# AHupuJR/REFID

Measured on AMD Instinct MI355X. Metric: interpolated frames/sec (train step) GoPro 256x256 11+1, higher is better.
Workload: dtype f32

## Files before the change

### refid_amd/csrc/wgrad_wino24.hip

```cpp
#include "common.h"
#include "wgrad_args.h"
#include <cstdlib>
#include <cstring>
#include <type_traits>
#include <vector>

#ifndef REFID_W24_ABLATE
#define REFID_W24_ABLATE 0
#endif
#define W24_NO_DMA (REFID_W24_ABLATE == 1 || REFID_W24_ABLATE == 5 || REFID_W24_ABLATE == 6)
#define W24_NO_MFMA (REFID_W24_ABLATE == 2)
#define W24_NO_LDS (REFID_W24_ABLATE == 3 || REFID_W24_ABLATE == 6)
#define W24_NO_BAR (REFID_W24_ABLATE == 4 || REFID_W24_ABLATE == 5 || REFID_W24_ABLATE == 6)

namespace {

__device__ __forceinline__ float w24_fake(float seed) { asm volatile("" : "+v"(seed)); return seed; }

constexpr int IT = 32;
constexpr int TC = 4;
constexpr int GH = 4, GW = 4 * TC;
constexpr int XH = GH + 2, XW = GW + 2;
constexpr int X_BYTES = XH * XW * IT * 4;
constexpr int GS_BYTES = GH * GW * 32 * 4;
// ... 288 lines not shown
        }
    };
    switch (wave) {
        case 0: kloop(std::integral_constant<int, 0>{}); break;
        case 1: kloop(std::integral_constant<int, 1>{}); break;
        case 2: kloop(std::integral_constant<int, 2>{}); break;
        default: kloop(std::integral_constant<int, 3>{}); break;
    }

#pragma unroll
    for (int j = 0; j < 6; ++j) {
        float* sl = a.slabs + ((long long)((split * (DOWN ? 4 : 1) + phase) * NXI + wave * 6 + j) * a.CoP) * a.CiP;
#pragma unroll
        for (int sm = 0; sm < NS; ++sm) {
            const int co = co0 + sm * 32 + li;
#pragma unroll
            for (int qd = 0; qd < 4; ++qd) {
                const int ci = ci0 + 8 * qd + 4 * kh;
                f32x4 vv;
#pragma unroll
                for (int k = 0; k < 4; ++k) vv[k] = acc[j][sm][4 * qd + k];
                f32x4* dst = reinterpret_cast<f32x4*>(sl + (long long)co * a.CiP + ci);
                if (a.accum) vv += *dst;
                *dst = vv;
            }
        }
    }
    if (a.bslabs != nullptr && blockIdx.y == 0 && phase == 0 && wave == 1) {
#pragma unroll
        for (int sm = 0; sm < NS; ++sm) {
            const float tot = bs[sm] + __shfl_xor(bs[sm], 32, 64);
            if (kh == 0) {
                float* dst = a.bslabs + (long long)split * a.CoP + co0 + sm * 32 + li;
                *dst = a.accum ? *dst + tot : tot;
            }
        }
    }
}

constexpr int PAIR_STAGES = 3;
constexpr int PAIR_G0 = 2 * PAIR_STAGES * X_BYTES;
constexpr int PAIR_LDS_BYTES = PAIR_G0 + PAIR_STAGES * 2 * GS_BYTES;

__device__ __forceinline__ int w24_lane_again() {
    int l = __builtin_amdgcn_mbcnt_hi(~0u, __builtin_amdgcn_mbcnt_lo(~0u, 0u));
    asm volatile("" : "+v"(l));
    return l;
}

template <bool DOWN>
__global__ __launch_bounds__(512, 1) void wgrad_wino24_pair_kernel(const W24Args a) {
    constexpr int NS = 2, OT = 32 * NS, XPS = DOWN ? 2 : 1;
    extern __shared__ __attribute__((aligned(16))) char smem[];
    const int tid = threadIdx.x, lane = tid & 63;
    const int wave = __builtin_amdgcn_readfirstlane(tid >> 6);
    const int row = wave & 3, hf = wave >> 2;
    const int li = lane & 31, kh = lane >> 5;
    const int phase = DOWN ? blockIdx.z / a.ncoT : 0, php = phase >> 1, phq = phase & 1;
    const int co0 = (DOWN ? blockIdx.z % a.ncoT : blockIdx.z) * OT, ci0 = (2 * blockIdx.y + hf) * IT;
    const int split = blockIdx.x;
    const int Hin = DOWN ? a.Hin : a.H, Win = DOWN ? a.Win : a.W;

    const bool xFromA = ci0 < a.Ca || ci0 >= a.Ctot;
    const int xld = xFromA ? a.ldA : a.ldB;
    const long long gpixAll = (long long)a.N * a.Ho * a.Wo, xpixAll = (long long)a.N * Hin * Win;
    const int limG = (int)min(gpixAll * a.ldG * 4, 0x7fffffffLL), limX = (int)min(xpixAll * xld * 4, 0x7fffffffLL);
    const int ntAll = a.ntiles * a.groups;
    const int chunk = (ntAll + a.nsplit - 1) / a.nsplit;
    const int p0 = min(split * chunk, ntAll), p1 = min(p0 + chunk, ntAll);

    int qg, qn, qy, qx;
    {
        int t = p0 < ntAll ? p0 : 0;
        qg = t / a.ntiles; t -= qg * a.ntiles;
        qx = t % a.tilesX; t /= a.tilesX;
        qy = t % a.tilesY; qn = t / a.tilesY;
    }
    const int xq = ci0 + (lane & 7) * 4, xt = ci0 + (lane & 31), gq = co0 + (lane & 7) * 4;
    const int xlc = ((lane >> 3) * XPS * xld + (xFromA ? xq : xq - a.Ca)) * 4;
    const int xlt = ((lane >> 5) * XPS * xld + (xFromA ? xt : xt - a.Ca)) * 4;
    const int glc = ((lane >> 3) * a.ldG + gq) * 4;
    const bool fullch = ci0 + IT <= a.Ctot && co0 + OT <= a.Co;
    constexpr int OOB = 0x7ff00000;
    const int xRowB = XPS * Win * xld * 4, gRowB = a.Wo * a.ldG * 4;
    auto x_origin = [&](int n, int ty, int tx) {
        return ((n * Hin + XPS * (ty * GH - a.pad) + php) * Win + XPS * (tx * GW - a.pad) + phq) * xld * 4;
    };
    const float* gPtr = a.g[qg];
    const float* xPtr = xFromA ? a.inA[qg] : a.inB[qg];
    int xTile = x_origin(qn, qy, qx);
    int gTile = ((qn * a.Ho + qy * GH) * a.Wo + qx * GW) * a.ldG * 4;
    const int xr0 = row < 2 ? 2 * row : row + 2, nxr = row < 2 ? 2 : 1;
    const int gr0 = 2 * (row - 2);
    auto request = [&](int st) {
        const int oy0 = qy * GH, ox0 = qx * GW;
        const int iy0 = oy0 - a.pad, ix0 = ox0 - a.pad;
        const __amdgpu_buffer_rsrc_t rsG = __builtin_amdgcn_make_buffer_rsrc(const_cast<float*>(gPtr), 0, limG, 0x00020000);
        const __amdgpu_buffer_rsrc_t rsX = __builtin_amdgcn_make_buffer_rsrc(const_cast<float*>(xPtr), 0, limX, 0x00020000);
        char* xdst = smem + (hf * PAIR_STAGES + st) * X_BYTES;
        char* gdst = smem + PAIR_G0 + st * (2 * GS_BYTES) + hf * GS_BYTES;
        const bool fast = fullch && ix0 >= 0 && ix0 + XW <= a.W && ox0 + GW <= a.Wo && xld * 8 * XPS * 4 < 0x100000 && a.ldG * 8 * 4 < 0x100000;
        if (fast) {
#pragma unroll
            for (int k = 0; k < 2; ++k) {
                if (k < nxr && !W24_NO_DMA) {
                    const int r = xr0 + k;
                    const int base = (unsigned)(iy0 + r) < (unsigned)a.H ? xTile + r * xRowB : OOB;
                    char* dst = xdst + r * (XW * IT * 4);
                    __builtin_amdgcn_raw_ptr_buffer_load_lds(rsX, (lds_ptr24)dst, 16, base + xlc, 0, 0, 0);
                    __builtin_amdgcn_raw_ptr_buffer_load_lds(rsX, (lds_ptr24)(dst + 1024), 16, base + 8 * XPS * xld * 4 + xlc, 0, 0, 0);
                    __builtin_amdgcn_raw_ptr_buffer_load_lds(rsX, (lds_ptr24)(dst + 2048), 4, base + 16 * XPS * xld * 4 + xlt, 0, 0, 0);
                }
            }
#pragma unroll
            for (int k = 0; k < 2; ++k) {
                if (row >= 2 && !W24_NO_DMA) {
                    const int r = gr0 + k;
                    const int base = oy0 + r < a.Ho ? gTile + r * gRowB + hf * 128 : OOB;
                    char* dst = gdst + r * (GW * 32 * 4);
                    __builtin_amdgcn_raw_ptr_buffer_load_lds(rsG, (lds_ptr24)dst, 16, base + glc, 0, 0, 0);
                    __builtin_amdgcn_raw_ptr_buffer_load_lds(rsG, (lds_ptr24)(dst + 1024), 16, base + 8 * a.ldG * 4 + glc, 0, 0, 0);
                }
            }
        } else {
            const int l8 = lane >> 3, l32 = lane >> 5;
            const int xbadq = xq < a.Ctot ? 0 : -1, xbadt = xt < a.Ctot ? 0 : -1;
            const int gbad = gq + hf * 32 < a.Co ? 0 : -1;
            const int cx0 = (unsigned)(ix0 + l8) < (unsigned)a.W ? 0 : -1;
            const int cx1 = (unsigned)(ix0 + 8 + l8) < (unsigned)a.W ? 0 : -1;
            const int cxt = (unsigned)(ix0 + 16 + l32) < (unsigned)a.W ? 0 : -1;
            const int cg0 = ox0 + l8 < a.Wo ? 0 : -1, cg1 = ox0 + 8 + l8 < a.Wo ? 0 : -1;
#pragma unroll
            for (int k = 0; k < 2; ++k) {
                if (k < nxr && !W24_NO_DMA) {
                    const int r = xr0 + k;
                    const int rbad = (unsigned)(iy0 + r) < (unsigned)a.H ? 0 : -1;
                    const int base = xTile + r * xRowB;
                    char* dst = xdst + r * (XW * IT * 4);
                    __builtin_amdgcn_raw_ptr_buffer_load_lds(rsX, (lds_ptr24)dst, 16, (base + xlc) | xbadq | rbad | cx0, 0, 0, 0);
                    __builtin_amdgcn_raw_ptr_buffer_load_lds(rsX, (lds_ptr24)(dst + 1024), 16,
                                                             (base + 8 * XPS * xld * 4 + xlc) | xbadq | rbad | cx1, 0, 0, 0);
                    __builtin_amdgcn_raw_ptr_buffer_load_lds(rsX, (lds_ptr24)(dst + 2048), 4,
                                                             (base + 16 * XPS * xld * 4 + xlt) | xbadt | rbad | cxt, 0, 0, 0);
                }
            }
#pragma unroll
            for (int k = 0; k < 2; ++k) {
                if (row >= 2 && !W24_NO_DMA) {
                    const int r = gr0 + k;
                    const int rbad = oy0 + r < a.Ho ? 0 : -1;
                    const int base = gTile + r * gRowB + hf * 128;
                    char* dst = gdst + r * (GW * 32 * 4);
                    __builtin_amdgcn_raw_ptr_buffer_load_lds(rsG, (lds_ptr24)dst, 16, (base + glc) | gbad | rbad | cg0, 0, 0, 0);
                    __builtin_amdgcn_raw_ptr_buffer_load_lds(rsG, (lds_ptr24)(dst + 1024), 16,
                                                             (base + 8 * a.ldG * 4 + glc) | gbad | rbad | cg1, 0, 0, 0);
                }
            }
        }
        if (REFID_W24_ABLATE == 7) return;
        qx += 1;
        if (qx != a.tilesX) {
            xTile += GW * XPS * xld * 4;
            gTile += GW * a.ldG * 4;
        } else {
            qx = 0;
            qy += 1;
            if (qy == a.tilesY) {
                qy = 0;
                qn += 1;
                if (qn == a.N) {
                    qn = 0;
                    qg = min(qg + 1, a.groups - 1);
                    gPtr = a.g[qg];
                    xPtr = xFromA ? a.inA[qg] : a.inB[qg];
                }
            }
            xTile = x_origin(qn, qy, 0);
            gTile = (qn * a.Ho + qy * GH) * a.Wo * a.ldG * 4;
        }
    };

    f32x16 acc[6][NS];
#pragma unroll
    for (int j = 0; j < 6; ++j)
#pragma unroll
        for (int sm = 0; sm < NS; ++sm)
#pragma unroll
            for (int r = 0; r < 16; ++r) acc[j][sm][r] = 0.f;

    static_assert(X_BYTES % 256 == 0 && (PAIR_STAGES * X_BYTES) / 256 < 256 && (PAIR_STAGES * 2 * GS_BYTES) / 256 < 256,
                  "ds_read2st64 offset range");
    lds_cf24* xe = (lds_cf24*)(smem + hf * PAIR_STAGES * X_BYTES) + (2 * kh) * (XW * IT) + li;
    lds_cf24* ge = (lds_cf24*)(smem + PAIR_G0) + (2 * kh) * (GW * 32) + li;
    lds_cf24* xb[4] = {xe, xe + IT, xe + 2 * IT, xe + 3 * IT};
    lds_cf24* gb[4] = {ge, ge + 32, ge + 2 * 32, ge + 3 * 32};
    asm volatile("" : "+v"(xb[0]), "+v"(xb[1]), "+v"(xb[2]), "+v"(xb[3]), "+v"(xe));
    asm volatile("" : "+v"(gb[0]), "+v"(gb[1]), "+v"(gb[2]), "+v"(gb[3]));

    auto kloop = [&](auto TI) {
        constexpr int I = decltype(TI)::value;
        using R = W24Row<I>;
        float bs[NS];
#pragma unroll
        for (int sm = 0; sm < NS; ++sm) bs[sm] = 0.f;
        auto tile = [&](auto ST) {
            constexpr int XO = decltype(ST)::value * (X_BYTES / 4), GO = decltype(ST)::value * (2 * GS_BYTES / 4);
            lds_cf24* xbb[4] = {xb[0] + XO, xb[1] + XO, xb[2] + XO, xb[3] + XO};
            lds_cf24* gbb[4] = {gb[0] + GO, gb[1] + GO, gb[2] + GO, gb[3] + GO};
            f32x2 t[6], p4, p5;
#pragma unroll
            for (int s = 0; s < TC; s += 2) {
                R::x_rows(xbb, s, t);
                if (s == 0) {
                    const f32x2 a01 = R::x_rows01(xe + XO);
                    t[0] = w24_pair<0, 0>(a01, t[4]);
                    t[1] = w24_pair<1, 0>(a01, t[5]);
                } else {
                    t[0] = w24_pair<1, 0>(p4, t[4]);
                    t[1] = w24_pair<1, 0>(p5, t[5]);
                }
                p4 = t[4]; p5 = t[5];
                f32x2 v[6];
                R::v_cols(t, v);
#pragma unroll
                for (int sm = 0; sm < NS; ++sm) {
                    f32x2 x[4], z[6];
                    R::g_rows(gbb, s, sm, x);
                    R::z_cols(x, z);
                    if constexpr (I == 1) bs[sm] += z[1][0] + z[1][1];
#pragma unroll
                    for (int h = 0; h < 2; ++h)
#pragma unroll
                        for (int j = 0; j < 6; ++j) {
                            if (W24_NO_MFMA) { asm volatile("" :: "v"(v[j][h]), "v"(z[j][h])); continue; }
                            acc[j][sm] = __builtin_amdgcn_mfma_f32_32x32x2f32(v[j][h], z[j][h], acc[j][sm], 0, 0, 0);
                        }
                }
            }
        };
        const int n = p1 - p0;
        auto step = [&](auto ST, int j) {
            constexpr int S = decltype(ST)::value;
            if (j + 1 < n) __builtin_amdgcn_s_waitcnt(I < 2 ? 0x0F76 : 0x0F77);
            else __builtin_amdgcn_s_waitcnt(0x0F70);
            if (!W24_NO_BAR) __builtin_amdgcn_s_barrier();
            __builtin_amdgcn_sched_barrier(0);
            if (j + 2 < n) request((S + 2) % PAIR_STAGES);
            tile(ST);
        };
        if (n > 0) request(0);
        if (n > 1) request(1);
        int j = 0;
        for (; j + 3 <= n; j += 3) {
            step(std::integral_constant<int, 0>{}, j);
            step(std::integral_constant<int, 1>{}, j + 1);
            step(std::integral_constant<int, 2>{}, j + 2);
        }
        if (j < n) {
            step(std::integral_constant<int, 0>{}, j);
            if (j + 1 < n) step(std::integral_constant<int, 1>{}, j + 1);
        }
        if constexpr (I == 1) {
            if (a.bslabs != nullptr && blockIdx.y == 0 && hf == 0 && phase == 0) {
                const int le = w24_lane_again();
#pragma unroll
                for (int sm = 0; sm < NS; ++sm) {
                    const float tot = bs[sm] + __shfl_xor(bs[sm], 32, 64);
                    if ((le >> 5) == 0) {
                        float* dst = a.bslabs + (long long)split * a.CoP + co0 + sm * 32 + (le & 31);
                        *dst = a.accum ? *dst + tot : tot;
                    }
                }
            }
        }
    };
    switch (row) {
        case 0: kloop(std::integral_constant<int, 0>{}); break;
        case 1: kloop(std::integral_constant<int, 1>{}); break;
        case 2: kloop(std::integral_constant<int, 2>{}); break;
        default: kloop(std::integral_constant<int, 3>{}); break;
    }

    const int le = w24_lane_again(), lie = le & 31, khe = le >> 5;
#pragma unroll
    for (int j = 0; j < 6; ++j) {
        float* sl = a.slabs + ((long long)((split * (DOWN ? 4 : 1) + phase) * NXI + row * 6 + j) * a.CoP) * a.CiP;
#pragma unroll
        for (int sm = 0; sm < NS; ++sm) {
            const int co = co0 + sm * 32 + lie;
#pragma unroll
            for (int qd = 0; qd < 4; ++qd) {
                const int ci = ci0 + 8 * qd + 4 * khe;
                f32x4 vv;
#pragma unroll
                for (int k = 0; k < 4; ++k) vv[k] = acc[j][sm][4 * qd + k];
                f32x4* dst = reinterpret_cast<f32x4*>(sl + (long long)co * a.CiP + ci);
                if (a.accum) vv += *dst;
                *dst = vv;
            }
        }
    }
}

struct W24rArgs {
    const float* slabs; const float* bslabs; float* dw; float* db;
    int nsplit, Co, Ci, CoP, CiP, iBase, iTotal, perGroup;
    int nsplitW;
    int down;
};

__device__ __forceinline__ void w24_fold_body(const float* __restrict__ slabs, float* __restrict__ part, long long slabFloats,
                                              int nsplit, int S, int piece, int s) {
    const long long off = ((long long)piece * 256 + threadIdx.x) * 4;
    if (off >= slabFloats) return;
    const f32x4* p = reinterpret_cast<const f32x4*>(slabs + off);
    const long long st4 = slabFloats / 4;
    f32x4 a0 = {0.f, 0.f, 0.f, 0.f}, a1 = a0;
    int k = s;
    for (; k + S < nsplit; k += 2 * S) { a0 += p[k * st4]; a1 += p[(k + S) * st4]; }
    if (k < nsplit) a0 += p[k * st4];
    *reinterpret_cast<f32x4*>(part + (long long)s * slabFloats + off) = a0 + a1;
}
__global__ __launch_bounds__(256) void wgrad_wino24_fold_kernel(const float* __restrict__ slabs, float* __restrict__ part,
                                                                long long slabFloats, int nsplit, int S) {
    w24_fold_body(slabs, part, slabFloats, nsplit, S, blockIdx.x, blockIdx.y);
}

constexpr int FOLD_BATCH = 96;
struct FoldJob { const float* slabs; float* part; long long slabFloats; int nsplit, S; };
struct FoldBatch { FoldJob job[FOLD_BATCH]; int blk0[FOLD_BATCH + 1]; int n; };
static_assert(sizeof(FoldBatch) <= 4096, "kernel-argument block");
__global__ __launch_bounds__(256) void wgrad_fold_batch_kernel(const FoldBatch b) {
    int j = 0;
    for (int k = 1; k < b.n; ++k) j = (int)blockIdx.x >= b.blk0[k] ? k : j;
    const FoldJob& f = b.job[j];
    const int blk = (int)blockIdx.x - b.blk0[j];
    const int pieces = (int)((f.slabFloats / 4 + 255) / 256);
    w24_fold_body(f.slabs, f.part, f.slabFloats, f.nsplit, f.S, blk % pieces, blk / pieces);
}
thread_local std::vector<FoldJob> fold_queue;

__device__ __forceinline__ void w24_reduce_body(const W24rArgs& a, const int blk, float* part) {
    const long long plane = (long long)a.CoP * a.CiP;
    const long long slabStride = NXI * plane;
    const int lpe = a.perGroup, eb = 256 / lpe;
    const int el = threadIdx.x % eb, sub = threadIdx.x / eb;
    const long long e = (long long)blk * eb + el;
    const bool live = e < (long long)a.Co * a.Ci;
    const int ci = live ? (int)(e % a.Ci) : 0, co = live ? (int)(e / a.Ci) : 0;
    {
        const float* p = a.slabs + (long long)co * a.CiP + ci;
        float u[NXI];
#pragma unroll
        for (int x = 0; x < NXI; ++x) u[x] = 0.f;
        if (live) {
            for (int k = sub; k < a.nsplitW; k += lpe) {
#pragma unroll
                for (int x = 0; x < NXI; ++x) u[x] += p[k * slabStride + x * plane];
            }
        }
        if (lpe > 1) {
#pragma unroll
            for (int x = 0; x < NXI; ++x) part[threadIdx.x * (NXI + 1) + x] = u[x];
            __syncthreads();
            if (sub == 0) {
                for (int s2 = 1; s2 < lpe; ++s2) {
#pragma unroll
                    for (int x = 0; x < NXI; ++x) u[x] += part[(s2 * eb + el) * (NXI + 1) + x];
                }
            }
        }
        if (live && sub == 0) {
            constexpr float c4 = 0.25f, c6 = 1.f / 6.f, c12 = 1.f / 12.f, c24 = 1.f / 24.f;
            float dg[9];
#pragma unroll
            for (int pp = 0; pp < 3; ++pp) {
                float t[6];
#pragma unroll
                for (int j = 0; j < 6; ++j) {
                    const float m = 0.5f * (u[6 + j] + u[12 + j]), d = 0.5f * (u[6 + j] - u[12 + j]);
                    t[j] = pp == 0 ? u[j] + m : (pp == 1 ? d : m + u[18 + j]);
                }
                const float s12 = t[1] + t[2], d21 = t[2] - t[1], s34 = t[3] + t[4], d34 = t[3] - t[4];
                dg[pp * 3 + 0] = c4 * t[0] - c6 * s12 + c24 * s34;
                dg[pp * 3 + 1] = c6 * d21 + c12 * d34;
                dg[pp * 3 + 2] = c6 * (s34 - s12) + t[5];
            }
            float* dst = a.dw + ((long long)co * a.iTotal + a.iBase + ci) * 9;
#pragma unroll
            for (int k = 0; k < 9; ++k) dst[k] += dg[k];
        }
    }
    if (a.db != nullptr && blk == 0) {
        for (int c2 = threadIdx.x; c2 < a.Co; c2 += 256) {
            float s = 0.f;
            for (int k = 0; k < a.nsplit; ++k) s += a.bslabs[(long long)k * a.CoP + c2];
            a.db[c2] += s;
        }
    }
}

__global__ __launch_bounds__(256) void wgrad_wino24_reduce_kernel(const W24rArgs a) {
    __shared__ float part[256 * (NXI + 1)];
    w24_reduce_body(a, blockIdx.x, part);
}

__device__ __forceinline__ void w24_reduce_down_body(const W24rArgs& a, const int blk) {
    const long long plane = (long long)a.CoP * a.CiP;
    const long long slabStride = 4 * NXI * plane;
    const long long gid = (long long)blk * 256 + threadIdx.x;
    const long long e = gid >> 2;
    const int ph = (int)(gid & 3);
    const bool live = e < (long long)a.Co * a.Ci;
    const int ci = live ? (int)(e % a.Ci) : 0, co = live ? (int)(e / a.Ci) : 0;
    if (live) {
        const float* p = a.slabs + (long long)co * a.CiP + ci + ph * NXI * plane;
        float u[NXI];
#pragma unroll
        for (int x = 0; x < NXI; ++x) u[x] = 0.f;
        for (int k = 0; k < a.nsplitW; ++k) {
#pragma unroll
            for (int x = 0; x < NXI; ++x) u[x] += p[k * slabStride + x * plane];
        }
        constexpr float c4 = 0.25f, c6 = 1.f / 6.f, c12 = 1.f / 12.f, c24 = 1.f / 24.f;
        float* dst = a.dw + ((long long)co * a.iTotal + a.iBase + ci) * 16;
#pragma unroll
        for (int pp = 0; pp < 3; ++pp) {
            const int ky = 2 * pp + (ph >> 1) - 1;
            float t[6];
#pragma unroll
            for (int j = 0; j < 6; ++j) {
                const float m = 0.5f * (u[6 + j] + u[12 + j]), d = 0.5f * (u[6 + j] - u[12 + j]);
                t[j] = pp == 0 ? u[j] + m : (pp == 1 ? d : m + u[18 + j]);
            }
            const float s12 = t[1] + t[2], d21 = t[2] - t[1], s34 = t[3] + t[4], d34 = t[3] - t[4];
            const float r3[3] = {c4 * t[0] - c6 * s12 + c24 * s34, c6 * d21 + c12 * d34, c6 * (s34 - s12) + t[5]};
            if (ky < 0 || ky > 3) continue;
#pragma unroll
            for (int q = 0; q < 3; ++q) {
                const int kx = 2 * q + (ph & 1) - 1;
                if (kx >= 0 && kx <= 3) dst[ky * 4 + kx] += r3[q];
            }
        }
    }
    if (a.db != nullptr && blk == 0) {
        for (int c2 = threadIdx.x; c2 < a.Co; c2 += 256) {
            float sacc = 0.f;
            for (int k = 0; k < a.nsplit; ++k) sacc += a.bslabs[(long long)k * a.CoP + c2];
            a.db[c2] += sacc;
        }
    }
}

__global__ __launch_bounds__(256) void wgrad_wino24_reduce_down_kernel(const W24rArgs a) { w24_reduce_down_body(a, blockIdx.x); }

struct W24rBatch { W24rArgs job[REFID_FINISH_BATCH]; int blk0[REFID_FINISH_BATCH + 1]; int n; };
static_assert(sizeof(W24rBatch) <= 4096, "kernel-argument block");
__global__ __launch_bounds__(256) void wgrad_wino24_reduce_batch_kernel(const W24rBatch b) {
    __shared__ float part[256 * (NXI + 1)];
    int j = 0;
    for (int k = 1; k < b.n; ++k) j = (int)blockIdx.x >= b.blk0[k] ? k : j;
    const int blk = (int)blockIdx.x - b.blk0[j];
    if (b.job[j].down) w24_reduce_down_body(b.job[j], blk);
    else w24_reduce_body(b.job[j], blk, part);
}

struct W24rQueued { W24rArgs r; int nblocks; };
thread_local std::vector<W24rQueued> w24_queue;

struct Geo24 { int ncoT, nciT, tilesX, tilesY, ntiles, nsplit, CoP, CiP; };

int ns_of(const refid_wgrad_desc* d) { return d->c_o <= 32 ? 1 : 2; }
bool is_down(const refid_wgrad_desc* d) { return d->kh == 4; }

Geo24 geo24_of(const refid_wgrad_desc* d) {
    Geo24 g;
    const int OT = 32 * ns_of(d);
    g.ncoT = cdiv(d->c_o, OT);
    const int ci_geo = (d->phase != 0) ? d->i_total - d->i_base : d->c_a + d->c_b;
    g.nciT = cdiv(ci_geo > d->c_a + d->c_b ? ci_geo : d->c_a + d->c_b, IT);
    g.tilesX = cdiv(d->wo, GW);
    g.tilesY = cdiv(d->ho, GH);
    g.ntiles = g.tilesX * g.tilesY * d->n;
    const char* wgsEnv = getenv("REFID_W24_WGS");
    const int wgs = wgsEnv ? atoi(wgsEnv) : 512;
    int want = cdiv(ns_of(d) == 1 ? wgs * 3 / 2 : wgs, g.ncoT * g.nciT * (is_down(d) ? 4 : 1));
    if (want >= 8) want = want / 8 * 8;
    if (want < 1) want = 1;
    if (want > g.ntiles) want = g.ntiles;
    g.nsplit = want;
    g.CoP = g.ncoT * OT;
    g.CiP = g.nciT * IT;
    return g;
}

int pair_mode() { const char* e = getenv("REFID_W24_PAIR"); return e ? atoi(e) : 1; }
bool pair_fits(const refid_wgrad_desc* d, const Geo24& g) { return ns_of(d) == 2 && g.nciT % 2 == 0; }

}

int refid_slab_fold_count(long long slabFloats, int nsplit) {
    if (nsplit < 2) return 0;
    const long long pieces = (slabFloats / 4 + 255) / 256;
    int S = (int)((2048 + pieces - 1) / pieces);
    if (S > 16) S = 16;
    if (S >= nsplit) S = nsplit / 2;
    return S < 1 ? 1 : S;
}
int refid_launch_slab_fold(const float* slabs, float* part, long long slabFloats, int nsplit, int S, hipStream_t st) {
    static const bool batch_folds = !(getenv("REFID_FOLD_BATCH") && getenv("REFID_FOLD_BATCH")[0] == '0');
    if (batch_folds && refid_finish_defer_now()) {
        fold_queue.push_back({slabs, part, slabFloats, nsplit, S});
        return 0;
    }
    hipLaunchKernelGGL(wgrad_wino24_fold_kernel, dim3((unsigned)((slabFloats / 4 + 255) / 256), S), dim3(256), 0, st, slabs, part,
                       slabFloats, nsplit, S);
    REFID_LAUNCH_CHECK("wgrad_slab_fold");
    return 0;
}

int refid_slab_fold_flush(hipStream_t st) {
    size_t at = 0;
    while (at < fold_queue.size()) {
        FoldBatch b;
        memset(&b, 0, sizeof(b));
        int n = 0;
        long long blk = 0;
        for (; n < FOLD_BATCH && at < fold_queue.size(); ++n, ++at) {
            const FoldJob& f = fold_queue[at];
            const long long nb = ((f.slabFloats / 4 + 255) / 256) * f.S;
            if (n > 0 && blk + nb > 0x3fffffffLL) break;
            b.job[n] = f;
            b.blk0[n] = (int)blk;
            blk += nb;
        }
        b.blk0[n] = (int)blk; b.n = n;
        hipLaunchKernelGGL(wgrad_fold_batch_kernel, dim3((unsigned)blk), dim3(256), 0, st, b);
        if (hipGetLastError() != hipSuccess) { fold_queue.clear(); refid_set_error("wgrad_fold_batch: launch failed"); return 1; }
    }
    fold_queue.clear();
    return 0;
}

int refid_wino24_finish_flush(hipStream_t st) {
    size_t at = 0;
    while (at < w24_queue.size()) {
        W24rBatch b;
        memset(&b, 0, sizeof(b));
        int n = 0, blk = 0;
        for (; n < REFID_FINISH_BATCH && at < w24_queue.size(); ++n, ++at) {
            b.job[n] = w24_queue[at].r;
            b.blk0[n] = blk;
            blk += w24_queue[at].nblocks;
        }
        b.blk0[n] = blk; b.n = n;
        hipLaunchKernelGGL(wgrad_wino24_reduce_batch_kernel, dim3(blk), dim3(256), 0, st, b);
        if (hipGetLastError() != hipSuccess) { w24_queue.clear(); refid_set_error("wgrad_wino24_reduce_batch: launch failed"); return 1; }
    }
    w24_queue.clear();
    return 0;
}

namespace {
long long slab_floats(const refid_wgrad_desc* d, const Geo24& g) { return (long long)(is_down(d) ? 4 : 1) * NXI * g.CoP * g.CiP; }
}

size_t refid_wgrad_wino24_workspace_bytes(const refid_wgrad_desc* d) {
    const Geo24 g = geo24_of(d);
    const long long slab = slab_floats(d, g);
    return ((size_t)g.nsplit * slab + (size_t)g.nsplit * g.CoP + (size_t)refid_slab_fold_count(slab, g.nsplit) * slab) * sizeof(float);
}

int refid_wgrad_wino24_launch(const refid_wgrad_desc* d, hipStream_t st) {
    static std::atomic<unsigned long long> attr_done{0}, attr_done1{0}, attr_done2{0}, attr_done3{0};
    if (int rc = refid_lds_attr_once(attr_done, &wgrad_wino24_kernel<2, false>, lds24_bytes(2), "wgrad_wino24")) return rc;
    if (int rc = refid_lds_attr_once(attr_done1, &wgrad_wino24_kernel<1, false>, lds24_bytes(1), "wgrad_wino24<1>")) return rc;
    if (int rc = refid_lds_attr_once(attr_done2, &wgrad_wino24_kernel<2, true>, lds24_bytes(2), "wgrad_wino24<down>")) return rc;
    if (int rc = refid_lds_attr_once(attr_done3, &wgrad_wino24_kernel<1, true>, lds24_bytes(1), "wgrad_wino24<1, down>")) return rc;
    static std::atomic<unsigned long long> attr_done4{0}, attr_done5{0};
    if (int rc = refid_lds_attr_once(attr_done4, &wgrad_wino24_pair_kernel<false>, PAIR_LDS_BYTES, "wgrad_wino24<pair>")) return rc;
    if (int rc = refid_lds_attr_once(attr_done5, &wgrad_wino24_pair_kernel<true>, PAIR_LDS_BYTES, "wgrad_wino24<pair, down>")) return rc;
    const Geo24 g = geo24_of(d);
    const bool down = is_down(d);
    const long long slab = slab_floats(d, g);
    const int pmode = pair_mode();
    const bool pair = pmode != 0 && pair_fits(d, g);
    REFID_CHECK(pair || pmode != 2, "wgrad (Winograd 2x4 tiles): REFID_W24_PAIR=2, but this launch takes the four-wave form "
                                    "(c_o <= 32 or an odd number of input-channel tiles)");
    if (down)
        REFID_CHECK(d->kw == 4 && d->stride == 2 && d->pad == 1 && d->h % 2 == 0 && d->w % 2 == 0 && d->ho == d->h / 2 && d->wo == d->w / 2,
                    "wgrad (algo 7): a 4x4 stride-2 pad-1 conv over an even-sized input");
    REFID_CHECK(d->c_b == 0 || d->c_a % IT == 0, "wgrad (Winograd 2x4 tiles): c_a must be a multiple of %d for two sources", IT);
    REFID_CHECK(d->ld_g % 4 == 0 && d->ld_a % 4 == 0 && (d->c_b == 0 || d->ld_b % 4 == 0) && d->c_o % 4 == 0 &&
                    d->c_a % 4 == 0 && d->c_b % 4 == 0,
                "wgrad (Winograd 2x4 tiles): pitches and channel counts must be multiples of 4 floats (16-byte LDS-DMA pieces)");
    {
        const long long lim = 0x7fffffffLL;
        REFID_CHECK((long long)d->n * d->ho * d->wo * d->ld_g * 4 < lim && (long long)d->n * d->h * d->w * d->ld_a * 4 < lim &&
                        (d->c_b == 0 || (long long)d->n * d->h * d->w * d->ld_b * 4 < lim),
                    "wgrad (Winograd 2x4 tiles): tensor too large for 32-bit buffer offsets (use algo 0)");
    }
    W24Args a;
    const int ngrp = d->groups > 1 ? d->groups : 1;
    REFID_CHECK(ngrp <= REFID_WGRAD_MAX_GROUPS, "wgrad: at most %d grouped time steps", REFID_WGRAD_MAX_GROUPS);
    for (int k = 0; k < REFID_WGRAD_MAX_GROUPS; ++k) {
        const bool on = k > 0 && k < ngrp;
        a.g[k] = k == 0 ? d->g : (on ? d->g_more[k - 1] : d->g);
        a.inA[k] = k == 0 ? d->in_a : (on ? d->in_a_more[k - 1] : d->in_a);
        a.inB[k] = k == 0 ? d->in_b : (on ? d->in_b_more[k - 1] : d->in_b);
        REFID_CHECK(a.g[k] && a.inA[k] && (d->c_b == 0 || a.inB[k]), "wgrad: null tensor pointer in group %d", k);
        REFID_CHECK(((uintptr_t)a.g[k] | (uintptr_t)a.inA[k] | (uintptr_t)(d->c_b ? a.inB[k] : nullptr)) % 16 == 0,
                    "wgrad (Winograd 2x4 tiles): tensors must be 16-byte aligned (group %d)", k);
    }
    a.groups = ngrp;
    a.ldG = d->ld_g; a.Co = d->c_o;
    a.ldA = d->ld_a; a.ldB = d->ld_b;
    a.Ca = d->c_a; a.Ctot = d->c_a + d->c_b;
    a.slabs = d->slabs;
    a.bslabs = d->db ? d->slabs + (size_t)g.nsplit * slab : nullptr;
    a.N = d->n; a.H = d->h; a.W = d->w; a.Ho = d->ho; a.Wo = d->wo; a.pad = d->pad;
    a.Hin = d->h; a.Win = d->w; a.ncoT = g.ncoT;
    if (down) { a.H = d->ho; a.W = d->wo; a.pad = 1; }
    a.tilesX = g.tilesX; a.tilesY = g.tilesY; a.ntiles = g.ntiles; a.nsplit = g.nsplit;
    a.CoP = g.CoP; a.CiP = g.CiP;
    a.accum = (d->phase == 2);
    if (d->phase != 3) {
        if (pair) {
            if (down)
                hipLaunchKernelGGL((wgrad_wino24_pair_kernel<true>), dim3(g.nsplit, g.nciT / 2, 4 * g.ncoT), dim3(512), PAIR_LDS_BYTES, st, a);
            else
                hipLaunchKernelGGL((wgrad_wino24_pair_kernel<false>), dim3(g.nsplit, g.nciT / 2, g.ncoT), dim3(512), PAIR_LDS_BYTES, st, a);
        } else if (down) {
            if (ns_of(d) == 1)
                hipLaunchKernelGGL((wgrad_wino24_kernel<1, true>), dim3(g.nsplit, g.nciT, 4 * g.ncoT), dim3(256), lds24_bytes(1), st, a);
            else
                hipLaunchKernelGGL((wgrad_wino24_kernel<2, true>), dim3(g.nsplit, g.nciT, 4 * g.ncoT), dim3(256), lds24_bytes(2), st, a);
        } else if (ns_of(d) == 1)
            hipLaunchKernelGGL((wgrad_wino24_kernel<1, false>), dim3(g.nsplit, g.nciT, g.ncoT), dim3(256), lds24_bytes(1), st, a);
        else
            hipLaunchKernelGGL((wgrad_wino24_kernel<2, false>), dim3(g.nsplit, g.nciT, g.ncoT), dim3(256), lds24_bytes(2), st, a);
        REFID_LAUNCH_CHECK("wgrad_wino24");
    }
    if (d->phase == 1 || d->phase == 2) return 0;
    W24rArgs r;
    r.slabs = a.slabs; r.bslabs = a.bslabs; r.dw = d->dw; r.db = d->db;
    r.nsplit = g.nsplit; r.Co = d->o_real;
    int nred = g.nsplit;
    if (const int S = refid_slab_fold_count(slab, g.nsplit)) {
        const long long slabFloats = slab;
        float* part = d->slabs + (size_t)g.nsplit * slab + (size_t)g.nsplit * g.CoP;
        if (int rc = refid_launch_slab_fold(a.slabs, part, slabFloats, g.nsplit, S, st)) return rc;
        r.slabs = part;
        nred = S;
    }
    r.Ci = (d->phase == 0 && a.Ctot < d->i_total - d->i_base) ? a.Ctot : d->i_total - d->i_base;
    r.CoP = g.CoP; r.CiP = g.CiP; r.iBase = d->i_base; r.iTotal = d->i_total;
    const long long total = (long long)r.Co * r.Ci;
    int lpe = 1;
    while (lpe < 16 && (long long)lpe * 2 * total <= 65536 && lpe * 2 <= nred) lpe *= 2;
    r.perGroup = lpe;
    r.nsplitW = nred;
    r.down = down ? 1 : 0;
    if (refid_finish_defer_now()) {
        for (const W24rQueued& q : w24_queue)
            if (q.r.dw == r.dw && q.r.iBase == r.iBase) {
                if (int rc = refid_slab_fold_flush(st)) return rc;
                if (int rc = refid_wino24_finish_flush(st)) return rc;
                break;
            }
        w24_queue.push_back({r, down ? (int)((total * 4 + 255) / 256) : (int)((total + 256 / lpe - 1) / (256 / lpe))});
        return 0;
    }
    if (down) {
        hipLaunchKernelGGL(wgrad_wino24_reduce_down_kernel, dim3((int)((total * 4 + 255) / 256)), dim3(256), 0, st, r);
        REFID_LAUNCH_CHECK("wgrad_wino24_reduce_down");
        return 0;
    }
    hipLaunchKernelGGL(wgrad_wino24_reduce_kernel, dim3((int)((total + 256 / lpe - 1) / (256 / lpe))), dim3(256), 0, st, r);
    REFID_LAUNCH_CHECK("wgrad_wino24_reduce");
    return 0;
}
```

Measured before the change: 506.8.

## Add dedicated Winograd kernel and reduce path for stride-2 4x4 down-conv weight grads

Adds a separate weight-gradient kernel for the 4x4 stride-2 downsampling convolution. It uses a different Winograd decomposition with 6-row output tiles, 20 transform points and its own input/gradient transforms, plus a matching reduce body that inverts the transform into the 4x4 kernel taps. It is enabled by default through REFID_W24_DOWN and bypasses the pair kernel for these layers. The aim is fewer MFMA and transform operations per down-conv tile, paid for with a new code path, a different slab layout, a larger workspace and some numerical risk.

```diff
diff --git a/refid_amd/csrc/wgrad_wino24.hip b/refid_amd/csrc/wgrad_wino24.hip
--- a/refid_amd/csrc/wgrad_wino24.hip
+++ b/refid_amd/csrc/wgrad_wino24.hip
@@ -614,6 +614,296 @@
     }
 }
 
+constexpr int DGH = 6, DXH = DGH + 1;
+constexpr int DX_BYTES = DXH * XW * IT * 4;
+constexpr int DGS_BYTES = DGH * GW * 32 * 4;
+constexpr int down_lds_bytes(int ns) { return 2 * (DX_BYTES + ns * DGS_BYTES); }
+constexpr int NXD = 20;
+
+template <int I>
+struct W24DownRow {
+    using B = W24Row<I>;
+    static constexpr int XR = XW * IT, GR = GW * 32, GSUB = DGH * GW * 32;
+    static __device__ __forceinline__ void x_rows(lds_cf24* const (&xb)[4], int s, f32x2 (&t)[5]) {
+#pragma unroll
+        for (int c = 0; c < 4; ++c) {
+            const int col = 4 * s + 1 + c;
+            lds_cf24* p = xb[col & 3] + (col & ~3) * IT;
+            const f32x2 a = f32x2{p[B::XA * XR], p[B::XA * XR + 4 * IT]};
+            const f32x2 b = f32x2{p[B::XB * XR], p[B::XB * XR + 4 * IT]};
+            t[1 + c] = B::x_comb(a, b);
+        }
+    }
+    static __device__ __forceinline__ float x_row0(lds_cf24* xe) { return B::x_comb(xe[B::XA * XR], xe[B::XB * XR]); }
+    static __device__ __forceinline__ void g_rows(lds_cf24* const (&gb)[4], int s, int sub, f32x2 (&x)[4]) {
+#pragma unroll
+        for (int c = 0; c < 4; ++c) {
+            const int col = 4 * s + c;
+            lds_cf24* p = gb[col & 3] + sub * GSUB + (col & ~3) * 32;
+            if constexpr (I == 0) x[c] = f32x2{p[0], p[4 * 32]};
+            else if constexpr (I == 3) x[c] = f32x2{p[2 * GR], p[2 * GR + 4 * 32]};
+            else {
+                const f32x2 g0 = f32x2{p[0], p[4 * 32]}, g1 = f32x2{p[GR], p[GR + 4 * 32]}, g2 = f32x2{p[2 * GR], p[2 * GR + 4 * 32]};
+                x[c] = I == 1 ? (g0 + g2) + g1 : (g0 + g2) - g1;
+            }
+        }
+    }
+    static __device__ __forceinline__ void v_cols(const f32x2 (&t)[5], f32x2 (&v)[5]) {
+        const f32x2 d31 = t[3] - t[1];
+        v[0] = 2.f * (t[0] - t[2]) + d31;
+        v[1] = (t[3] - t[2]) - 2.f * t[1];
+        v[2] = 2.f * t[1] + (-3.f * t[2] + t[3]);
+        v[3] = d31;
+        v[4] = (t[4] - t[2]) - 2.f * d31;
+    }
+    static __device__ __forceinline__ void z_cols(const f32x2 (&x)[4], f32x2 (&z)[5]) {
+        const f32x2 e = x[0] + x[2], o = x[1] + x[3], e4 = 4.f * x[2] + x[0], o4 = 4.f * x[3] + x[1];
+        z[0] = x[0]; z[1] = e + o; z[2] = e - o; z[3] = 2.f * o4 + e4; z[4] = x[3];
+    }
+};
+
+template <int NS>
+__global__ __launch_bounds__(256, 2) void wgrad_wino24_down_kernel(const W24Args a) {
+    constexpr int OT = 32 * NS, XPS = 2;
+    constexpr int G0 = 2 * DX_BYTES, GST_BYTES = NS * DGS_BYTES;
+    extern __shared__ __attribute__((aligned(16))) char smem[];
+    const int tid = threadIdx.x, lane = tid & 63;
+    const int wave = __builtin_amdgcn_readfirstlane(tid >> 6);
+    const int li = lane & 31, kh = lane >> 5;
+    const int phase = blockIdx.z / a.ncoT, php = phase >> 1, phq = phase & 1;
+    const int co0 = (blockIdx.z % a.ncoT) * OT, ci0 = blockIdx.y * IT;
+    const int split = blockIdx.x;
+    const int Hin = a.Hin, Win = a.Win;
+
+    const bool xFromA = ci0 < a.Ca || ci0 >= a.Ctot;
+    const int xld = xFromA ? a.ldA : a.ldB;
+    const long long gpixAll = (long long)a.N * a.Ho * a.Wo, xpixAll = (long long)a.N * Hin * Win;
+    const int limG = (int)min(gpixAll * a.ldG * 4, 0x7fffffffLL), limX = (int)min(xpixAll * xld * 4, 0x7fffffffLL);
+    const int ntAll = a.ntiles * a.groups;
+    const int chunk = (ntAll + a.nsplit - 1) / a.nsplit;
+    const int p0 = min(split * chunk, ntAll), p1 = min(p0 + chunk, ntAll);
+
+    int qg, qn, qy, qx;
+    {
+        int t = p0 < ntAll ? p0 : 0;
+        qg = t / a.ntiles; t -= qg * a.ntiles;
+        qx = t % a.tilesX; t /= a.tilesX;
+        qy = t % a.tilesY; qn = t / a.tilesY;
+    }
+    const int xq = ci0 + (lane & 7) * 4, xt = ci0 + (lane & 31), gq = co0 + (lane & 7) * 4;
+    const int xlc = ((lane >> 3) * XPS * xld + (xFromA ? xq : xq - a.Ca)) * 4;
+    const int xlt = ((lane >> 5) * XPS * xld + (xFromA ? xt : xt - a.Ca)) * 4;
+    const int glc = ((lane >> 3) * a.ldG + gq) * 4;
+    const bool fullch = ci0 + IT <= a.Ctot && co0 + OT <= a.Co;
+    constexpr int OOB = 0x7ff00000;
+    const int xRowB = XPS * Win * xld * 4, gRowB = a.Wo * a.ldG * 4;
+    auto x_origin = [&](int n, int ty, int tx) {
+        return ((n * Hin + XPS * (ty * DGH - php) + php) * Win + XPS * (tx * GW - phq) + phq) * xld * 4;
+    };
+    const float* gPtr = a.g[qg];
+    const float* xPtr = xFromA ? a.inA[qg] : a.inB[qg];
+    int xTile = x_origin(qn, qy, qx);
+    int gTile = ((qn * a.Ho + qy * DGH) * a.Wo + qx * GW) * a.ldG * 4;
+    const int q0 = NS == 2 ? 3 * wave : wave, nq = NS == 2 ? 3 : (wave < 3 ? 1 : 3);
+    auto request = [&](int buf) {
+        const int oy0 = qy * DGH, ox0 = qx * GW;
+        const int iy0 = oy0 - php, ix0 = ox0 - phq;
+        const __amdgpu_buffer_rsrc_t rsG = __builtin_amdgcn_make_buffer_rsrc(const_cast<float*>(gPtr), 0, limG, 0x00020000);
+        const __amdgpu_buffer_rsrc_t rsX = __builtin_amdgcn_make_buffer_rsrc(const_cast<float*>(xPtr), 0, limX, 0x00020000);
+        char* xdst = smem + buf * DX_BYTES;
+        char* gdst = smem + G0 + buf * GST_BYTES;
+        const bool fast = fullch && ix0 >= 0 && ix0 + XW - 1 <= a.W && ox0 + GW <= a.Wo && xld * 8 * XPS * 4 < 0x100000 && a.ldG * 8 * 4 < 0x100000;
+        if (fast) {
+#pragma unroll
+            for (int k = 0; k < 2; ++k) {
+                const int r = wave + 4 * k;
+                if (r < DXH) {
+                    const int base = (unsigned)(iy0 + r) < (unsigned)a.H ? xTile + r * xRowB : OOB;
+                    char* dst = xdst + r * (XW * IT * 4);
+                    __builtin_amdgcn_raw_ptr_buffer_load_lds(rsX, (lds_ptr24)dst, 16, base + xlc, 0, 0, 0);
+                    __builtin_amdgcn_raw_ptr_buffer_load_lds(rsX, (lds_ptr24)(dst + 1024), 16, base + 8 * XPS * xld * 4 + xlc, 0, 0, 0);
+                    __builtin_amdgcn_raw_ptr_buffer_load_lds(rsX, (lds_ptr24)(dst + 2048), 4, base + 16 * XPS * xld * 4 + xlt, 0, 0, 0);
+                }
+            }
+#pragma unroll
+            for (int k = 0; k < 3; ++k) {
+                if (k < nq) {
+                    const int q = q0 + k, r = q % DGH, sub = q / DGH;
+                    const int base = oy0 + r < a.Ho ? gTile + r * gRowB + sub * 128 : OOB;
+                    char* dst = gdst + sub * DGS_BYTES + r * (GW * 32 * 4);
+                    __builtin_amdgcn_raw_ptr_buffer_load_lds(rsG, (lds_ptr24)dst, 16, base + glc, 0, 0, 0);
+                    __builtin_amdgcn_raw_ptr_buffer_load_lds(rsG, (lds_ptr24)(dst + 1024), 16, base + 8 * a.ldG * 4 + glc, 0, 0, 0);
+                }
+            }
+        } else {
+            const int l8 = lane >> 3, l32 = lane >> 5;
+            const int xbadq = xq < a.Ctot ? 0 : -1, xbadt = xt < a.Ctot ? 0 : -1;
+            const int gbad0 = gq < a.Co ? 0 : -1, gbad1 = gq + 32 < a.Co ? 0 : -1;
+            const int cx0 = (unsigned)(ix0 + l8) < (unsigned)a.W ? 0 : -1;
+            const int cx1 = (unsigned)(ix0 + 8 + l8) < (unsigned)a.W ? 0 : -1;
+            const int cxt = (unsigned)(ix0 + 16 + l32) < (unsigned)a.W ? 0 : -1;
+            const int cg0 = ox0 + l8 < a.Wo ? 0 : -1, cg1 = ox0 + 8 + l8 < a.Wo ? 0 : -1;
+#pragma unroll
+            for (int k = 0; k < 2; ++k) {
+                const int r = wave + 4 * k;
+                if (r < DXH) {
+                    const int rbad = (unsigned)(iy0 + r) < (unsigned)a.H ? 0 : -1;
+                    const int base = xTile + r * xRowB;
+                    char* dst = xdst + r * (XW * IT * 4);
+                    __builtin_amdgcn_raw_ptr_buffer_load_lds(rsX, (lds_ptr24)dst, 16, (base + xlc) | xbadq | rbad | cx0, 0, 0, 0);
+                    __builtin_amdgcn_raw_ptr_buffer_load_lds(rsX, (lds_ptr24)(dst + 1024), 16,
+                                                             (base + 8 * XPS * xld * 4 + xlc) | xbadq | rbad | cx1, 0, 0, 0);
+                    __builtin_amdgcn_raw_ptr_buffer_load_lds(rsX, (lds_ptr24)(dst + 2048), 4,
+                                                             (base + 16 * XPS * xld * 4 + xlt) | xbadt | rbad | cxt, 0, 0, 0);
+                }
+            }
+#pragma unroll
+            for (int k = 0; k < 3; ++k) {
+                if (k < nq) {
+                    const int q = q0 + k, r = q % DGH, sub = q / DGH;
+                    const int rbad = oy0 + r < a.Ho ? 0 : -1;
+                    const int base = gTile + r * gRowB + sub * 128;
+                    const int gbad = sub ? gbad1 : gbad0;
+                    char* dst = gdst + sub * DGS_BYTES + r * (GW * 32 * 4);
+                    __builtin_amdgcn_raw_ptr_buffer_load_lds(rsG, (lds_ptr24)dst, 16, (base + glc) | gbad | rbad | cg0, 0, 0, 0);
+                    __builtin_amdgcn_raw_ptr_buffer_load_lds(rsG, (lds_ptr24)(dst + 1024), 16,
+                                                             (base + 8 * a.ldG * 4 + glc) | gbad | rbad | cg1, 0, 0, 0);
+                }
+            }
+        }
+        qx += 1;
+        if (qx != a.tilesX) {
+            xTile += GW * XPS * xld * 4;
+            gTile += GW * a.ldG * 4;
+        } else {
+            qx = 0;
+            qy += 1;
+            if (qy == a.tilesY) {
+                qy = 0;
+                qn += 1;
+                if (qn == a.N) {
+                    qn = 0;
+                    qg = min(qg + 1, a.groups - 1);
+                    gPtr = a.g[qg];
+                    xPtr = xFromA ? a.inA[qg] : a.inB[qg];
+                }
+            }
+            xTile = x_origin(qn, qy, 0);
+            gTile = (qn * a.Ho + qy * DGH) * a.Wo * a.ldG * 4;
+        }
+    };
+
+    f32x16 acc[5][NS];
+#pragma unroll
+    for (int j = 0; j < 5; ++j)
+#pragma unroll
+        for (int sm = 0; sm < NS; ++sm)
+#pragma unroll
+            for (int r = 0; r < 16; ++r) acc[j][sm][r] = 0.f;
+    float bs[NS];
+#pragma unroll
+    for (int sm = 0; sm < NS; ++sm) bs[sm] = 0.f;
+
+    static_assert(DX_BYTES % 256 == 0 && DGS_BYTES % 256 == 0 && (DX_BYTES + 3 * XW * IT * 4 + 16 * IT * 4) / 256 < 256 &&
+                      (GST_BYTES + NS * DGS_BYTES) / 256 < 256, "ds_read2st64 offset range");
+    lds_cf24* xe = (lds_cf24*)smem + (3 * kh) * (XW * IT) + li;
+    lds_cf24* ge = (lds_cf24*)(smem + G0) + (3 * kh) * (GW * 32) + li;
+    lds_cf24* xb[4] = {xe, xe + IT, xe + 2 * IT, xe + 3 * IT};
+    lds_cf24* gb[4] = {ge, ge + 32, ge + 2 * 32, ge + 3 * 32};
+    asm volatile("" : "+v"(xb[0]), "+v"(xb[1]), "+v"(xb[2]), "+v"(xb[3]), "+v"(xe));
+    asm volatile("" : "+v"(gb[0]), "+v"(gb[1]), "+v"(gb[2]), "+v"(gb[3]));
+
+    auto kloop = [&](auto TI) {
+        constexpr int I = decltype(TI)::value;
+        using R = W24DownRow<I>;
+        auto tile = [&](auto BUF) {
+            constexpr int XO = decltype(BUF)::value * (DX_BYTES / 4), GO = decltype(BUF)::value * (GST_BYTES / 4);
+            lds_cf24* xbb[4] = {xb[0] + XO, xb[1] + XO, xb[2] + XO, xb[3] + XO};
+            lds_cf24* gbb[4] = {gb[0] + GO, gb[1] + GO, gb[2] + GO, gb[3] + GO};
+            f32x2 t[5], p4;
+#pragma unroll
+            for (int s = 0; s < TC; s += 2) {
+                R::x_rows(xbb, s, t);
+                if (s == 0) {
+                    const float c0 = R::x_row0(xe + XO);
+                    t[0] = w24_pair<0, 0>(f32x2{c0, c0}, t[4]);
+                } else {
+                    t[0] = w24_pair<1, 0>(p4, t[4]);
+                }
+                p4 = t[4];
+                f32x2 v[5];
+                R::v_cols(t, v);
+#pragma unroll
+                for (int sm = 0; sm < NS; ++sm) {
+                    f32x2 x[4], z[5];
+                    R::g_rows(gbb, s, sm, x);
+                    R::z_cols(x, z);
+                    if constexpr (I == 1) bs[sm] += z[1][0] + z[1][1];
+#pragma unroll
+                    for (int h = 0; h < 2; ++h)
+#pragma unroll
+                        for (int j = 0; j < 5; ++j)
+                            acc[j][sm] = __builtin_amdgcn_mfma_f32_32x32x2f32(v[j][h], z[j][h], acc[j][sm], 0, 0, 0);
+                }
+            }
+        };
+        auto sync = [&] {
+            __builtin_amdgcn_s_waitcnt(0x0F70);
+            __builtin_amdgcn_s_barrier();
+            __builtin_amdgcn_sched_barrier(0);
+        };
+        const int npairs = (p1 - p0) >> 1;
+        if (p0 < p1) request(0);
+        for (int i = 0; i < npairs; ++i) {
+            sync();
+            request(1);
+            tile(std::integral_constant<int, 0>{});
+            sync();
+            if (p0 + 2 * i + 2 < p1) request(0);
+            tile(std::integral_constant<int, 1>{});
+        }
+        if ((p1 - p0) & 1) {
+            sync();
+            tile(std::integral_constant<int, 0>{});
+        }
+    };
+    switch (wave) {
+        case 0: kloop(std::integral_constant<int, 0>{}); break;
+        case 1: kloop(std::integral_constant<int, 1>{}); break;
+        case 2: kloop(std::integral_constant<int, 2>{}); break;
+        default: kloop(std::integral_constant<int, 3>{}); break;
+    }
+
+#pragma unroll
+    for (int j = 0; j < 5; ++j) {
+        float* sl = a.slabs + ((long long)((split * 4 + phase) * NXD + wave * 5 + j) * a.CoP) * a.CiP;
+#pragma unroll
+        for (int sm = 0; sm < NS; ++sm) {
+            const int co = co0 + sm * 32 + li;
+#pragma unroll
+            for (int qd = 0; qd < 4; ++qd) {
+                const int ci = ci0 + 8 * qd + 4 * kh;
+                f32x4 vv;
+#pragma unroll
+                for (int k = 0; k < 4; ++k) vv[k] = acc[j][sm][4 * qd + k];
+                f32x4* dst = reinterpret_cast<f32x4*>(sl + (long long)co * a.CiP + ci);
+                if (a.accum) vv += *dst;
+                *dst = vv;
+            }
+        }
+    }
+    if (a.bslabs != nullptr && blockIdx.y == 0 && phase == 0 && wave == 1) {
+#pragma unroll
+        for (int sm = 0; sm < NS; ++sm) {
+            const float tot = bs[sm] + __shfl_xor(bs[sm], 32, 64);
+            if (kh == 0) {
+                float* dst = a.bslabs + (long long)split * a.CoP + co0 + sm * 32 + li;
+                *dst = a.accum ? *dst + tot : tot;
+            }
+        }
+    }
+}
+
 struct W24rArgs {
     const float* slabs; const float* bslabs; float* dw; float* db;
     int nsplit, Co, Ci, CoP, CiP, iBase, iTotal, perGroup;
@@ -764,7 +1054,53 @@
     }
 }
 
-__global__ __launch_bounds__(256) void wgrad_wino24_reduce_down_kernel(const W24rArgs a) { w24_reduce_down_body(a, blockIdx.x); }
+__device__ __forceinline__ void w24_reduce_down23_body(const W24rArgs& a, const int blk) {
+    const long long plane = (long long)a.CoP * a.CiP;
+    const long long slabStride = 4 * NXD * plane;
+    const long long gid = (long long)blk * 256 + threadIdx.x;
+    const long long e = gid >> 2;
+    const int ph = (int)(gid & 3);
+    const bool live = e < (long long)a.Co * a.Ci;
+    const int ci = live ? (int)(e % a.Ci) : 0, co = live ? (int)(e / a.Ci) : 0;
+    if (live) {
+        const float* p = a.slabs + (long long)co * a.CiP + ci + ph * NXD * plane;
+        float u[NXD];
+#pragma unroll
+        for (int x = 0; x < NXD; ++x) u[x] = 0.f;
+        for (int k = 0; k < a.nsplitW; ++k) {
+#pragma unroll
+            for (int x = 0; x < NXD; ++x) u[x] += p[k * slabStride + x * plane];
+        }
+        constexpr float c6 = 1.f / 6.f;
+        float* dst = a.dw + ((long long)co * a.iTotal + a.iBase + ci) * 16;
+#pragma unroll
+        for (int pp = 0; pp < 2; ++pp) {
+            const int ky = 2 * pp + 1 - (ph >> 1);
+            float t[5];
+#pragma unroll
+            for (int j = 0; j < 5; ++j) {
+                const float m = 0.5f * (u[5 + j] + u[10 + j]), d = 0.5f * (u[5 + j] - u[10 + j]);
+                t[j] = pp == 0 ? u[j] + m : d + u[15 + j];
+            }
+            const float r2[2] = {0.5f * (t[0] - t[1]) + c6 * (t[3] - t[2]), (c6 * t[2] - 0.5f * t[1]) + (2.f * c6 * t[3] + t[4])};
+            const int kx = 1 - (ph & 1);
+            dst[ky * 4 + kx] += r2[0];
+            dst[ky * 4 + kx + 2] += r2[1];
+        }
+    }
+    if (a.db != nullptr && blk == 0) {
+        for (int c2 = threadIdx.x; c2 < a.Co; c2 += 256) {
+            float sacc = 0.f;
+            for (int k = 0; k < a.nsplit; ++k) sacc += a.bslabs[(long long)k * a.CoP + c2];
+            a.db[c2] += sacc;
+        }
+    }
+}
+
+__global__ __launch_bounds__(256) void wgrad_wino24_reduce_down_kernel(const W24rArgs a) {
+    if (a.down == 2) w24_reduce_down23_body(a, blockIdx.x);
+    else w24_reduce_down_body(a, blockIdx.x);
+}
 
 struct W24rBatch { W24rArgs job[REFID_FINISH_BATCH]; int blk0[REFID_FINISH_BATCH + 1]; int n; };
 static_assert(sizeof(W24rBatch) <= 4096, "kernel-argument block");
@@ -773,7 +1109,8 @@
     int j = 0;
     for (int k = 1; k < b.n; ++k) j = (int)blockIdx.x >= b.blk0[k] ? k : j;
     const int blk = (int)blockIdx.x - b.blk0[j];
-    if (b.job[j].down) w24_reduce_down_body(b.job[j], blk);
+    if (b.job[j].down == 2) w24_reduce_down23_body(b.job[j], blk);
+    else if (b.job[j].down) w24_reduce_down_body(b.job[j], blk);
     else w24_reduce_body(b.job[j], blk, part);
 }
 
@@ -785,14 +1122,20 @@
 int ns_of(const refid_wgrad_desc* d) { return d->c_o <= 32 ? 1 : 2; }
 bool is_down(const refid_wgrad_desc* d) { return d->kh == 4; }
 
-Geo24 geo24_of(const refid_wgrad_desc* d) {
+bool down_f23(const refid_wgrad_desc* d) {
+    if (!is_down(d)) return false;
+    const char* e = getenv("REFID_W24_DOWN");
+    return !e || atoi(e) != 0;
+}
+
+Geo24 geo24_of(const refid_wgrad_desc* d, bool f23) {
     Geo24 g;
     const int OT = 32 * ns_of(d);
     g.ncoT = cdiv(d->c_o, OT);
     const int ci_geo = (d->phase != 0) ? d->i_total - d->i_base : d->c_a + d->c_b;
     g.nciT = cdiv(ci_geo > d->c_a + d->c_b ? ci_geo : d->c_a + d->c_b, IT);
     g.tilesX = cdiv(d->wo, GW);
-    g.tilesY = cdiv(d->ho, GH);
+    g.tilesY = cdiv(d->ho, f23 ? DGH : GH);
     g.ntiles = g.tilesX * g.tilesY * d->n;
     const char* wgsEnv = getenv("REFID_W24_WGS");
     const int wgs = wgsEnv ? atoi(wgsEnv) : 512;
@@ -874,13 +1217,21 @@
 }
 
 namespace {
-long long slab_floats(const refid_wgrad_desc* d, const Geo24& g) { return (long long)(is_down(d) ? 4 : 1) * NXI * g.CoP * g.CiP; }
+long long slab_floats(const refid_wgrad_desc* d, const Geo24& g, bool f23) {
+    return (long long)(is_down(d) ? 4 : 1) * (f23 ? NXD : NXI) * g.CoP * g.CiP;
+}
+size_t workspace_bytes_of(const refid_wgrad_desc* d, bool f23) {
+    const Geo24 g = geo24_of(d, f23);
+    const long long slab = slab_floats(d, g, f23);
+    return ((size_t)g.nsplit * slab + (size_t)g.nsplit * g.CoP + (size_t)refid_slab_fold_count(slab, g.nsplit) * slab) * sizeof(float);
+}
 }
 
 size_t refid_wgrad_wino24_workspace_bytes(const refid_wgrad_desc* d) {
-    const Geo24 g = geo24_of(d);
-    const long long slab = slab_floats(d, g);
-    return ((size_t)g.nsplit * slab + (size_t)g.nsplit * g.CoP + (size_t)refid_slab_fold_count(slab, g.nsplit) * slab) * sizeof(float);
+    const size_t w = workspace_bytes_of(d, false);
+    if (!is_down(d)) return w;
+    const size_t w23 = workspace_bytes_of(d, true);
+    return w23 > w ? w23 : w;
 }
 
 int refid_wgrad_wino24_launch(const refid_wgrad_desc* d, hipStream_t st) {
@@ -892,12 +1243,15 @@
     static std::atomic<unsigned long long> attr_done4{0}, attr_done5{0};
     if (int rc = refid_lds_attr_once(attr_done4, &wgrad_wino24_pair_kernel<false>, PAIR_LDS_BYTES, "wgrad_wino24<pair>")) return rc;
     if (int rc = refid_lds_attr_once(attr_done5, &wgrad_wino24_pair_kernel<true>, PAIR_LDS_BYTES, "wgrad_wino24<pair, down>")) return rc;
-    const Geo24 g = geo24_of(d);
-    const bool down = is_down(d);
-    const long long slab = slab_floats(d, g);
+    static std::atomic<unsigned long long> attr_done6{0}, attr_done7{0};
+    if (int rc = refid_lds_attr_once(attr_done6, &wgrad_wino24_down_kernel<2>, down_lds_bytes(2), "wgrad_wino24_down")) return rc;
+    if (int rc = refid_lds_attr_once(attr_done7, &wgrad_wino24_down_kernel<1>, down_lds_bytes(1), "wgrad_wino24_down<1>")) return rc;
+    const bool down = is_down(d), f23 = down_f23(d);
+    const Geo24 g = geo24_of(d, f23);
+    const long long slab = slab_floats(d, g, f23);
     const int pmode = pair_mode();
-    const bool pair = pmode != 0 && pair_fits(d, g);
-    REFID_CHECK(pair || pmode != 2, "wgrad (Winograd 2x4 tiles): REFID_W24_PAIR=2, but this launch takes the four-wave form "
+    const bool pair = !f23 && pmode != 0 && pair_fits(d, g);
+    REFID_CHECK(pair || pmode != 2 || f23, "wgrad (Winograd 2x4 tiles): REFID_W24_PAIR=2, but this launch takes the four-wave form "
                                     "(c_o <= 32 or an odd number of input-channel tiles)");
     if (down)
         REFID_CHECK(d->kw == 4 && d->stride == 2 && d->pad == 1 && d->h % 2 == 0 && d->w % 2 == 0 && d->ho == d->h / 2 && d->wo == d->w / 2,
@@ -937,7 +1291,12 @@
     a.CoP = g.CoP; a.CiP = g.CiP;
     a.accum = (d->phase == 2);
     if (d->phase != 3) {
-        if (pair) {
+        if (f23) {
+            if (ns_of(d) == 1)
+                hipLaunchKernelGGL((wgrad_wino24_down_kernel<1>), dim3(g.nsplit, g.nciT, 4 * g.ncoT), dim3(256), down_lds_bytes(1), st, a);
+            else
+                hipLaunchKernelGGL((wgrad_wino24_down_kernel<2>), dim3(g.nsplit, g.nciT, 4 * g.ncoT), dim3(256), down_lds_bytes(2), st, a);
+        } else if (pair) {
             if (down)
                 hipLaunchKernelGGL((wgrad_wino24_pair_kernel<true>), dim3(g.nsplit, g.nciT / 2, 4 * g.ncoT), dim3(512), PAIR_LDS_BYTES, st, a);
             else
@@ -972,7 +1331,7 @@
     while (lpe < 16 && (long long)lpe * 2 * total <= 65536 && lpe * 2 <= nred) lpe *= 2;
     r.perGroup = lpe;
     r.nsplitW = nred;
-    r.down = down ? 1 : 0;
+    r.down = down ? (f23 ? 2 : 1) : 0;
     if (refid_finish_defer_now()) {
         for (const W24rQueued& q : w24_queue)
             if (q.r.dw == r.dw && q.r.iBase == r.iBase) {
```

After: 512.5 (median of 6 runs). 1.1% higher.
